# theivyzhang/droplet_visual_odometry

Hardware: AMD Instinct MI355X
Metric: frames/sec (detect+match+pose) at 1280×720, 2000 feats; ATE vs reference (higher is better)
Workload: dtype u8/f32/f64

## Files before the change

droplet_visual_odometry_amd/csrc/orb.hip:

```cpp
#include "dvo_internal.h"
#include "retain_best.h"

#include <climits>
#include <type_traits>

namespace dvo {

namespace {

__constant__ int8_t c_pattern[256 * 4] = {
#include "../../data/orb_bit_pattern_31.inc"
};
__constant__ __attribute__((aligned(16))) float c_pattern_f[256 * 4] = {
#include "../../data/orb_bit_pattern_31.inc"
};

constexpr int c_umax[16] = {15, 15, 15, 15, 14, 14, 14, 13, 13, 12, 11, 10, 9, 8, 6, 3};
struct IcTable {
    uint32_t w[4][32][10][2];
};
constexpr IcTable ic_table() {
    IcTable t{};
    for (int o = 0; o < 4; ++o)
        for (int r = 0; r < 31; ++r)
// ... 593 lines not shown
    const u16x2 Y = __builtin_elementwise_max(__builtin_elementwise_min(c0, c8), __builtin_elementwise_min(c4, c12));
    const u16x2 m = __builtin_elementwise_max(__builtin_elementwise_sub_sat(X, v), __builtin_elementwise_sub_sat(v, Y));
    return __builtin_bit_cast(uint32_t, __builtin_elementwise_sub_sat(m, as_u16x2(thr2)));
}
__device__ __forceinline__ uint32_t lane_prefix(unsigned long long bal) {
    return __builtin_amdgcn_mbcnt_hi((uint32_t)(bal >> 32), __builtin_amdgcn_mbcnt_lo((uint32_t)bal, 0u));
}
template <int kSeg>
__device__ __forceinline__ int seg_index(const int* cnt, int e) {
    int s = 0;
#pragma unroll
    for (int k = 0; k < 3; ++k) {
        const bool past = e >= cnt[k];
        e -= past ? cnt[k] : 0;
        s += past ? 1 : 0;
        if (!past) break;
    }
    return s * kSeg + e;
}
template <int kSeg>
__device__ __forceinline__ int seg_at(const uint16_t* list, const int* cnt, int e) {
    return list[seg_index<kSeg>(cnt, e)];
}
__global__ __launch_bounds__(kFastNT, DVO_FAST_WAVES_PER_EU) void fast_strip_kernel(StreamParams P, int nseg) {
    int it;
    const int f = xcd_frame_item(P.plan.total_strips * nseg, P.nframes, it);
    if (f >= P.nframes) return;
    const int strip = it / nseg, seg = it - strip * nseg;
    int l = 0;
    while (l + 1 < P.plan.nlevels && strip >= P.plan.L[l + 1].strip_base) ++l;
    const LevelGeom& G = P.plan.L[l];
    const int c = strip - G.strip_base;
    const int per_seg = (G.nbands + nseg - 1) / nseg;
    const int b_begin = seg * per_seg, b_end = min(G.nbands, b_begin + per_seg);
    if (b_begin >= b_end) return;
    const int w = G.w, h = G.h;
    const int xs = kBorder + c * kFastTW, xe = min(xs + kFastTW, w - kBorder);
    const int bx = xs - 7;
    const int thr = P.plan.fast_threshold;
    const uint8_t* src = level_ptr(P, f, l);
    const int sp = level_pitch(P, l);
    const auto rsrc = __builtin_amdgcn_make_buffer_rsrc(const_cast<uint8_t*>(src), 0, h * sp, 0x00020000);
    __shared__ __attribute__((aligned(16))) uint8_t img[kFtRows * kFtLW];
    __shared__ __attribute__((aligned(16))) uint8_t sc[(kBandRows + 2) * kFtLW];
    __shared__ uint16_t cand[4 * kFtSegCand + 256];
    __shared__ uint16_t wlist[4 * kFtWordCand + 256];
    __shared__ uint16_t carry[2][kFtCarryList];
    __shared__ int ncorner[4], ncarry[2];
    __shared__ uint32_t keep[kBandRows][4];
    __shared__ int row_off[4][kBandRows];
    const int lane = threadIdx.x & 63;
    const int wid = __builtin_amdgcn_readfirstlane(threadIdx.x >> 6);
    const int xlast = min(xe, w - 4);
    const int c_col = 4 + 4 * (lane & 31), c_hi = xlast - bx + 1 - c_col;
    const uint32_t c_vm = (c_col == 4 ? 0xFFFF0000u : 0xFFFFFFFFu) &
                          (c_hi >= 4 ? 0xFFFFFFFFu : c_hi <= 0 ? 0u : (1u << (8 * c_hi)) - 1u);
    const uint32_t c_vm4 = (c_vm & 1u) | ((c_vm >> 7) & 2u) | ((c_vm >> 14) & 4u) | ((c_vm >> 21) & 8u);
    const uint32_t thr2 = (uint32_t)thr * 0x10001u;
    uint32_t creg[kFtCarryR], pf[kFtPf], screg = 0;
    int voff[kFtPf];
#pragma unroll
    for (int k = 0; k < kFtPf; ++k) {
        const int q = threadIdx.x + k * kFastNT;
        const int rr = q / kFtWords, wd = q - rr * kFtWords;
        voff[k] = 4 * wd + rr * sp;
    }
    {
        const int ylo = kBorder + b_begin * kBandRows - 4;
#pragma unroll
        for (int k = 0; k < kFtCarryR; ++k) {
            const int q = threadIdx.x + k * kFastNT;
            creg[k] = q < kFtCarryW ? (uint32_t)__builtin_amdgcn_raw_buffer_load_b32(rsrc, voff[k], bx + ylo * sp, 0) : 0u;
        }
#pragma unroll
        for (int k = 0; k < kFtPf; ++k) {
            const int q = threadIdx.x + k * kFastNT;
            pf[k] = q < kFtNewW ? (uint32_t)__builtin_amdgcn_raw_buffer_load_b32(rsrc, voff[k], bx + (ylo + 8) * sp, 0) : 0u;
        }
    }
    if (threadIdx.x == 0) ncarry[0] = 0;
    for (int b = b_begin; b < b_end; ++b) {
        const int par = (b - b_begin) & 1;
        const int r0 = kBorder + b * kBandRows;
        const int r1 = min(r0 + kBandRows, h - kBorder);
        const int nrows = r1 - r0;
        const int item = G.band_base + b * G.ntx + c;
#pragma unroll
        for (int k = 0; k < kFtCarryR; ++k) {
            const int q = threadIdx.x + k * kFastNT;
            if (q < kFtCarryW) reinterpret_cast<uint32_t*>(img)[q] = creg[k];
        }
#pragma unroll
        for (int k = 0; k < kFtPf; ++k) {
            const int q = threadIdx.x + k * kFastNT;
            if (q < kFtNewW) reinterpret_cast<uint32_t*>(img)[kFtCarryW + q] = pf[k];
        }
        if (threadIdx.x < 2 * kFtWords) reinterpret_cast<uint32_t*>(sc)[threadIdx.x] = b == b_begin ? 0u : screg;
        for (int q = threadIdx.x; q < kBandRows * kFtLW / 16; q += kFastNT)
            reinterpret_cast<uint4*>(sc + 2 * kFtLW)[q] = make_uint4(0, 0, 0, 0);
        if (threadIdx.x < kBandRows * 4) keep[threadIdx.x >> 2][threadIdx.x & 3] = 0;
        if (threadIdx.x == 0) ncarry[par ^ 1] = 0;
        __syncthreads();
        if (b + 1 < b_end) {
#pragma unroll
            for (int k = 0; k < kFtCarryR; ++k) {
                const int q = threadIdx.x + k * kFastNT;
                creg[k] = q < kFtCarryW ? reinterpret_cast<const uint32_t*>(img)[kFtNewW + q] : 0u;
            }
            const int ynew = r0 + kBandRows + 4;
#pragma unroll
            for (int k = 0; k < kFtPf; ++k) {
                const int q = threadIdx.x + k * kFastNT;
                pf[k] = q < kFtNewW ? (uint32_t)__builtin_amdgcn_raw_buffer_load_b32(rsrc, voff[k], bx + ynew * sp, 0) : 0u;
            }
        }
        const int nsr = nrows + 2;
        const int sr_lo = b == b_begin ? 0 : 2;
        const int seg_off = wid * kFtSegCand, spare_i = 4 * kFtSegCand + wid * 64 + lane;
        int ncw = 0;
        {
            int n = 0, nw = 0;
            const int wl_off = wid * kFtWordCand, wl_spare = 4 * kFtWordCand + wid * 64 + lane;
            for (int sr = sr_lo + 2 * wid + (lane >> 5); __builtin_amdgcn_readfirstlane(sr - (lane >> 5)) < nsr;
                 sr += 8) {
                const int base = (sr + 3) * kFtLW + c_col;
                const uint32_t* wp = reinterpret_cast<const uint32_t*>(img + base);
                const uint32_t wc = wp[0], wl = wp[-1], wr = wp[1];
                const uint32_t wu = wp[-3 * kFtWords], wd = wp[3 * kFtWords];
                const uint32_t r0p = compass_pass(as_u16x2(__builtin_amdgcn_perm(0, wc, 0x0C020C00)),
                                                  as_u16x2(__builtin_amdgcn_perm(0, wu, 0x0C020C00)),
                                                  as_u16x2(__builtin_amdgcn_perm(0, wd, 0x0C020C00)),
                                                  as_u16x2(__builtin_amdgcn_perm(wr, wc, 0x0C050C03)),
                                                  as_u16x2(__builtin_amdgcn_perm(wc, wl, 0x0C030C01)), thr2);
                const uint32_t r1p = compass_pass(as_u16x2(__builtin_amdgcn_perm(0, wc, 0x0C030C01)),
                                                  as_u16x2(__builtin_amdgcn_perm(0, wu, 0x0C030C01)),
                                                  as_u16x2(__builtin_amdgcn_perm(0, wd, 0x0C030C01)),
                                                  as_u16x2(__builtin_amdgcn_perm(wr, wc, 0x0C060C04)),
                                                  as_u16x2(__builtin_amdgcn_perm(wc, wl, 0x0C040C02)), thr2);
                uint32_t b0, b1;
                asm("v_pk_min_u16 %0, %1, %2" : "=v"(b0) : "v"(r0p), "v"(0x00010001u));
                asm("v_pk_min_u16 %0, %1, %2" : "=v"(b1) : "v"(r1p), "v"(0x00010001u));
                const uint32_t m2 = b0 | (b1 << 1);
                const uint32_t msk = (m2 | (m2 >> 14)) & (sr < nsr ? c_vm4 : 0u);
                const bool any = msk != 0;
                const unsigned long long bal = __ballot(any);
                const int to = wl_off + nw + (int)lane_prefix(bal);
                wlist[any ? to : wl_spare] = (uint16_t)((base >> 2) | (msk << 12));
                nw += __popcll(bal);
            }
            __builtin_amdgcn_fence(__ATOMIC_RELEASE, "wavefront");
            __builtin_amdgcn_wave_barrier();
            __builtin_amdgcn_fence(__ATOMIC_ACQUIRE, "wavefront");
            for (int e0 = 0; e0 < nw; e0 += 64) {
                const int e = e0 + lane;
                const uint32_t ent = e < nw ? (uint32_t)wlist[wl_off + e] : 0u;
                const uint32_t msk = ent >> 12;
                const int a0 = (int)(ent & 0xFFFu) << 2;
                const uint32_t c = (uint32_t)__popc(msk);
                const unsigned long long b0 = __ballot(c & 1u), b1 = __ballot(c & 2u), b2 = __ballot(c & 4u);
                const int pre = n + (int)lane_prefix(b0) + 2 * (int)lane_prefix(b1) + 4 * (int)lane_prefix(b2);
#pragma unroll
                for (int k = 0; k < 4; ++k) {
                    const bool on = (msk >> k) & 1u;
                    const int to = seg_off + pre + __popc(msk & ((1u << k) - 1u));
                    if (on) cand[to] = (uint16_t)(a0 + k);
                }
                n += __popcll(b0) + 2 * __popcll(b1) + 4 * __popcll(b2);
            }
            __builtin_amdgcn_fence(__ATOMIC_RELEASE, "wavefront");
            __builtin_amdgcn_wave_barrier();
            __builtin_amdgcn_fence(__ATOMIC_ACQUIRE, "wavefront");
            for (int e0 = 0; e0 < n; e0 += 64) {
                const int e = e0 + lane;
                int a = 0, s = -1;
                if (e < n) {
                    a = cand[seg_off + e];
                    s = fast_score16_pk(img + a, kFtLW, thr);
                }
                const bool is_corner = s >= thr;
                if (is_corner) sc[a - 3 * kFtLW] = (uint8_t)s;
                const unsigned long long bal = __ballot(is_corner);
                cand[is_corner ? seg_off + ncw + (int)lane_prefix(bal) : spare_i] = (uint16_t)a;
                ncw += __popcll(bal);
            }
            if (lane == 0) ncorner[wid] = ncw;
        }
        __syncthreads();
        int cnt2[4];
#pragma unroll
        for (int k = 0; k < 4; ++k) cnt2[k] = ncorner[k];
        const int ncorners = cnt2[0] + cnt2[1] + cnt2[2] + cnt2[3];
        const int nc = ncarry[par];
        if (threadIdx.x < 2 * kFtWords) screg = reinterpret_cast<const uint32_t*>(sc)[kBandRows * kFtWords + threadIdx.x];
        for (int e = threadIdx.x; e < nc + ncorners; e += kFastNT) {
            const int a = (e < nc ? (int)carry[par][e] : seg_at<kFtSegCand>(cand, cnt2, e - nc)) -
                          3 * kFtLW;
            const int sr = a / kFtLW, x = bx + (a - sr * kFtLW);
            if (sr == kBandRows + 1) {
                const int slot = atomicAdd(&ncarry[par ^ 1], 1);
                carry[par ^ 1][slot] = (uint16_t)(a + 3 * kFtLW - kBandRows * kFtLW);
                continue;
            }
            if (sr < 1 || sr > nrows || x < xs || x >= xe) continue;
            const uint8_t* s = sc + a;
            const uint32_t v = s[0];
            const uint32_t nmax = max(max(max((uint32_t)s[-kFtLW - 1], (uint32_t)s[-kFtLW]),
                                          max((uint32_t)s[-kFtLW + 1], (uint32_t)s[-1])),
                                      max(max((uint32_t)s[1], (uint32_t)s[kFtLW - 1]),
                                          max((uint32_t)s[kFtLW], (uint32_t)s[kFtLW + 1])));
            if (v > nmax) {
                const int i_col = x - (xs - 1);
                atomicOr(&keep[sr - 1][i_col >> 5], 1u << (i_col & 31));
            }
        }
        __syncthreads();
        uint32_t* outp = P.buf.band_cand + (int64_t)f * P.plan.band_cand_stride + G.band_cand_off +
                         (int64_t)(b * G.ntx + c) * G.band_cap;
        {
            int rc = 0;
            if (lane < kBandRows && lane < nrows)
                rc = __popc(keep[lane][0]) + __popc(keep[lane][1]) + __popc(keep[lane][2]) + __popc(keep[lane][3]);
            int incl = rc;
#pragma unroll
            for (int o = 1; o < kBandRows; o <<= 1) {
                const int y2 = __shfl_up(incl, o);
                if (lane >= o) incl += y2;
            }
            if (lane < kBandRows) {
                row_off[wid][lane] = incl - rc;
                if (wid == 0)
                    P.buf.band_cnt[((int64_t)f * P.plan.total_bands + item) * kBandRows + lane] = ((incl - rc) << 16) | rc;
            }
            __builtin_amdgcn_fence(__ATOMIC_RELEASE, "wavefront");
            __builtin_amdgcn_wave_barrier();
            __builtin_amdgcn_fence(__ATOMIC_ACQUIRE, "wavefront");
        }
        for (int e = threadIdx.x; e < nc + ncorners; e += kFastNT) {
            const int a = (e < nc ? (int)carry[par][e] : seg_at<kFtSegCand>(cand, cnt2, e - nc)) - 3 * kFtLW;
            const int sr = a / kFtLW, x = bx + (a - sr * kFtLW);
            if (sr < 1 || sr > nrows || x < xs || x >= xe) continue;
            const int i_col = x - (xs - 1), wq = i_col >> 5;
            const uint32_t* kr = keep[sr - 1];
            if (!((kr[wq] >> (i_col & 31)) & 1)) continue;
            int before = __popc(kr[wq] & ((1u << (i_col & 31)) - 1));
            for (int q = 0; q < wq; ++q) before += __popc(kr[q]);
            outp[row_off[wid][sr - 1] + before] = ((uint32_t)sc[a] << 24) | ((uint32_t)(r0 + sr - 1) << 12) | (uint32_t)x;
        }
        __syncthreads();
    }
}

struct FastKeys {
    uint32_t* key;
    struct Elem {
        uint32_t k;
    };
    __device__ int val(int i) const { return (int)(key[i] >> 24); }
    __device__ void swap(int i, int j) const {
        uint32_t t = key[i];
        key[i] = key[j];
        key[j] = t;
    }
    __device__ Elem get(int i) const { return Elem{key[i]}; }
    __device__ void put(int i, Elem e) const { key[i] = e.k; }
    __device__ static int ev(Elem e) { return (int)(e.k >> 24); }
};

struct HarrisVals {
    float* v;
    uint32_t* key;
    struct Elem {
        float v;
        uint32_t k;
    };
    __device__ float val(int i) const { return v[i]; }
    __device__ void swap(int i, int j) const {
        float t = v[i];
        v[i] = v[j];
        v[j] = t;
        uint32_t u = key[i];
        key[i] = key[j];
        key[j] = u;
    }
    __device__ Elem get(int i) const { return Elem{v[i], key[i]}; }
    __device__ void put(int i, Elem e) const {
        v[i] = e.v;
        key[i] = e.k;
    }
    __device__ static float ev(Elem e) { return e.v; }
};

#ifndef DVO_SEL_NT
#define DVO_SEL_NT 128
#endif
constexpr int kSelNT = DVO_SEL_NT;
#ifndef DVO_SEL_NT0
#define DVO_SEL_NT0 256
#endif
constexpr int kSelNT0 = DVO_SEL_NT0;
#ifndef DVO_SEL_NT_CALL
#define DVO_SEL_NT_CALL 512
#endif
constexpr int kSelNTCall = DVO_SEL_NT_CALL, kSelCallFrames = 4;
constexpr int kSelLdsCap = 8192;
#ifndef DVO_SEL_LDS_CALL
#define DVO_SEL_LDS_CALL 1
#endif
constexpr bool kSelLdsCall = DVO_SEL_LDS_CALL != 0;

template <int NT, bool kLds>
__global__ __launch_bounds__(NT) void select_fast_kernel(StreamParams P, int l0) {
    const int l = l0 + blockIdx.x, f = blockIdx.y;
    if (l >= P.plan.nlevels) return;
    const LevelGeom& G = P.plan.L[l];
    __shared__ int lds[64];
    __shared__ int s_carry;
    const int32_t* rc = P.buf.band_cnt + ((int64_t)f * P.plan.total_bands + G.band_base) * kBandRows;
    const uint32_t* bsrc = P.buf.band_cand + (int64_t)f * P.plan.band_cand_stride + G.band_cand_off;
    uint32_t* A = P.buf.cand + (int64_t)f * P.plan.cand_stride + G.cand_off;
    if constexpr (kLds) {
        const int nseg = G.nbands * kBandRows * G.ntx;
        const int per = (nseg + NT - 1) / NT;
        const int s_begin = min(nseg, (int)threadIdx.x * per), s_end = min(nseg, s_begin + per);
        auto seg_word = [&](int sg) {
            const int cc = sg % G.ntx, br = sg / G.ntx;
            const int b = br / kBandRows, rr = br - b * kBandRows;
            const int tile = b * G.ntx + cc;
            return make_int2(tile, rc[(int64_t)tile * kBandRows + rr]);
        };
        constexpr int kG = 8;
        int mine = 0;
        for (int s0 = s_begin; s0 < s_end; s0 += kG) {
            int2 tv[kG];
#pragma unroll
            for (int k = 0; k < kG; ++k) tv[k] = s0 + k < s_end ? seg_word(s0 + k) : make_int2(0, 0);
#pragma unroll
            for (int k = 0; k < kG; ++k) mine += tv[k].y & 0xFFFF;
        }
        int tot;
        int o = block_excl_scan(mine, tot, lds);
        for (int s0 = s_begin; s0 < s_end; s0 += kG) {
            int2 tv[kG];
#pragma unroll
            for (int k = 0; k < kG; ++k) tv[k] = s0 + k < s_end ? seg_word(s0 + k) : make_int2(0, 0);
#pragma unroll
            for (int k = 0; k < kG; ++k) {
                const int cnt = tv[k].y & 0xFFFF, src_off = tv[k].x * G.band_cap + (tv[k].y >> 16);
                for (int i = 0; i < cnt; ++i) A[o + i] = bsrc[src_off + i];
                o += cnt;
            }
        }
        if (threadIdx.x == 0) s_carry = tot;
        __syncthreads();
    } else {
        const int nseg = G.nbands * kBandRows * G.ntx;
        if (threadIdx.x == 0) s_carry = 0;
        __syncthreads();
        for (int s0 = 0; s0 < nseg; s0 += NT) {
            const int sg = s0 + threadIdx.x;
            int cnt = 0, src_off = 0;
            if (sg < nseg) {
                const int cc = sg % G.ntx, br = sg / G.ntx;
                const int b = br / kBandRows, rr = br - b * kBandRows;
                const int tile = b * G.ntx + cc;
                const int v = rc[(int64_t)tile * kBandRows + rr];
                cnt = v & 0xFFFF;
                src_off = tile * G.band_cap + (v >> 16);
            }
            int tot;
            const int off = block_excl_scan(cnt, tot, lds);
            const int base = s_carry;
            for (int i = 0; i < cnt; ++i) A[base + off + i] = bsrc[src_off + i];
            __syncthreads();
            if (threadIdx.x == 0) s_carry = base + tot;
            __syncthreads();
        }
    }
    const int n = s_carry;
    __syncthreads();
    int32_t* Lpos = P.buf.sel_tmp + (int64_t)f * 2 * P.plan.cand_stride + 2 * G.cand_off;
    int32_t* Rasc = Lpos + G.cand_cap;
    int k;
    if constexpr (kLds) {
        __shared__ uint32_t s_key[kSelLdsCap];
        __shared__ int32_t s_L[kSelLdsCap], s_R[kSelLdsCap];
        if (n <= kSelLdsCap) {
            for (int i = threadIdx.x; i < n; i += NT) s_key[i] = A[i];
            __syncthreads();
            k = retain_best_block(FastKeys{s_key}, n, 2 * G.nper, -1, s_L, s_R, lds, P.plan.semantics);
            __syncthreads();
            for (int i = threadIdx.x; i < k; i += NT) A[i] = s_key[i];
        } else {
            k = retain_best_block(FastKeys{A}, n, 2 * G.nper, -1, Lpos, Rasc, lds, P.plan.semantics);
        }
    } else {
        k = retain_best_block(FastKeys{A}, n, 2 * G.nper, -1, Lpos, Rasc, lds, P.plan.semantics);
    }
    if (threadIdx.x == 0) P.buf.cnt1[f * kMaxLevels + l] = k;
}

#ifndef DVO_HARRIS_GROUPS
#define DVO_HARRIS_GROUPS 2
#endif
constexpr int kHG = DVO_HARRIS_GROUPS;
__host__ __device__ inline int harris_blocks_x(const Plan& pl) {
    int hb = 0;
    for (int l = 0; l < pl.nlevels; ++l) hb = hb > 2 * pl.L[l].nper ? hb : 2 * pl.L[l].nper;
    return (hb + 16 * kHG - 1) / (16 * kHG) + 1;
}

__global__ __launch_bounds__(256) void harris_kernel(StreamParams P) {
    __shared__ uint32_t win[kHG][16][32];
    const int l = blockIdx.y, f = blockIdx.z;
    const int hb = blockIdx.x, gdx = gridDim.x;
    const int n = P.buf.cnt1[f * kMaxLevels + l];
    const LevelGeom& G = P.plan.L[l];
    const uint8_t* img = level_ptr(P, f, l);
    const int step = level_pitch(P, l);
    const int lane = threadIdx.x & 63;
    const int wid = __builtin_amdgcn_readfirstlane(threadIdx.x >> 6);
    const int g = lane >> 4, j = lane & 15;
    const uint32_t* cand = P.buf.cand + (int64_t)f * P.plan.cand_stride + G.cand_off;
    float* resp = P.buf.resp + (int64_t)f * P.plan.cand_stride + G.cand_off;
    for (int base = (hb * 4 + wid) * 4 * kHG; base < n; base += gdx * 16 * kHG) {
        int x0[kHG], ax[kHG];
        uint32_t v0[kHG], v1[kHG];
#pragma unroll
        for (int u = 0; u < kHG; ++u) {
            const int i = min(base + 4 * u + g, n - 1);
            const uint32_t key = cand[i];
            x0[u] = key & 0xFFF;
            const int y0 = (key >> 12) & 0xFFF;
            ax[u] = (x0[u] - 4) & ~3;
            const uint8_t* wp = img + (int64_t)(y0 - 4) * step + ax[u];
            const int e1 = min(j + 16, 26);
            v0[u] = *reinterpret_cast<const uint32_t*>(wp + (int64_t)(j / 3) * step + 4 * (j % 3));
            v1[u] = *reinterpret_cast<const uint32_t*>(wp + (int64_t)(e1 / 3) * step + 4 * (e1 % 3));
        }
        __builtin_amdgcn_wave_barrier();
#pragma unroll
        for (int u = 0; u < kHG; ++u) {
            win[u][wid * 4 + g][j] = v0[u];
            win[u][wid * 4 + g][j + 16] = v1[u];
        }
        __builtin_amdgcn_wave_barrier();
#pragma unroll
        for (int u = 0; u < kHG; ++u) {
            const uint8_t* Wb = reinterpret_cast<const uint8_t*>(win[u][wid * 4 + g]);
            const int o = x0[u] - ax[u] - 3;
            int a = 0, b = 0, c = 0;
#pragma unroll
            for (int t = 0; t < 4; ++t) {
                const int pos = j + 16 * t;
                if (t < 3 || pos < 49) {
                    const int py = pos / 7, px = pos - 7 * py;
                    const uint8_t* q = Wb + (1 + py) * 12 + o + px;
                    const int Ix = (q[1] - q[-1]) * 2 + (q[-12 + 1] - q[-12 - 1]) + (q[12 + 1] - q[12 - 1]);
                    const int Iy = (q[12] - q[-12]) * 2 + (q[12 - 1] - q[-12 - 1]) + (q[12 + 1] - q[-12 + 1]);
                    a += Ix * Ix;
                    b += Iy * Iy;
                    c += Ix * Iy;
                }
            }
#pragma unroll
            for (int s2 = 8; s2 >= 1; s2 >>= 1) {
                a += __shfl_xor(a, s2);
                b += __shfl_xor(b, s2);
                c += __shfl_xor(c, s2);
            }
            if (j == 0 && base + 4 * u + g < n) {
                const float scale = 1.f / ((1 << 2) * 7 * 255.f);
                const float s4 = scale * scale * scale * scale;
                const float fa = (float)a, fb = (float)b, fc = (float)c;
                resp[base + 4 * u + g] = (fa * fb - fc * fc - 0.04f * (fa + fb) * (fa + fb)) * s4;
            }
        }
        __builtin_amdgcn_wave_barrier();
    }
}

template <int NT, bool kLds>
__global__ __launch_bounds__(NT) void select_harris_kernel(StreamParams P) {
    const int l = blockIdx.x, f = blockIdx.y;
    if (l >= P.plan.nlevels) return;
    const LevelGeom& G = P.plan.L[l];
    __shared__ int lds[64];
    const int n = P.buf.cnt1[f * kMaxLevels + l];
    uint32_t* A = P.buf.cand + (int64_t)f * P.plan.cand_stride + G.cand_off;
    float* R = P.buf.resp + (int64_t)f * P.plan.cand_stride + G.cand_off;
    int32_t* Lpos = P.buf.sel_tmp + (int64_t)f * 2 * P.plan.cand_stride + 2 * G.cand_off;
    int32_t* Rasc = Lpos + G.cand_cap;
    int k;
    if constexpr (kLds) {
        __shared__ float s_v[kSelLdsCap];
        __shared__ uint32_t s_key[kSelLdsCap];
        __shared__ int32_t s_L[kSelLdsCap], s_R[kSelLdsCap];
        if (n <= kSelLdsCap) {
            for (int i = threadIdx.x; i < n; i += NT) {
                s_v[i] = R[i];
                s_key[i] = A[i];
            }
            __syncthreads();
            k = retain_best_block(HarrisVals{s_v, s_key}, n, G.nper, -1, s_L, s_R, lds, P.plan.semantics);
            __syncthreads();
            for (int i = threadIdx.x; i < k; i += NT) {
                R[i] = s_v[i];
                A[i] = s_key[i];
            }
        } else {
            k = retain_best_block(HarrisVals{R, A}, n, G.nper, -1, Lpos, Rasc, lds, P.plan.semantics);
        }
    } else {
        k = retain_best_block(HarrisVals{R, A}, n, G.nper, -1, Lpos, Rasc, lds, P.plan.semantics);
    }
    if (threadIdx.x == 0) P.buf.cnt2[f * kMaxLevels + l] = k;
}

__device__ __forceinline__ float fast_atan2(float y, float x) {
    const float p1 = 0.9997878412794807f * (float)(180 / M_PI);
    const float p3 = -0.3258083974640975f * (float)(180 / M_PI);
    const float p5 = 0.1555786518463281f * (float)(180 / M_PI);
    const float p7 = -0.04432655554792128f * (float)(180 / M_PI);
    float ax = fabsf(x), ay = fabsf(y);
    float a, c, c2;
    if (ax >= ay) {
        c = ay / (ax + (float)2.220446049250313e-16);
        c2 = c * c;
        a = (((p7 * c2 + p5) * c2 + p3) * c2 + p1) * c;
    } else {
        c = ax / (ay + (float)2.220446049250313e-16);
        c2 = c * c;
        a = 90.f - (((p7 * c2 + p5) * c2 + p3) * c2 + p1) * c;
    }
    if (x < 0) a = 180.f - a;
    if (y < 0) a = 360.f - a;
    return a;
}

constexpr int kDPR = 19, kDPH = 2 * kDPR + 1, kDPW = 64;
#ifndef DVO_DKW
#define DVO_DKW 1
#endif
constexpr int kDKW = DVO_DKW;
constexpr int kDKB = 4 * kDKW;
constexpr int kICW = 36, kICR = 36;

constexpr int kDBRows = 8, kDBSeg = 5, kDBRaw = kDBRows + 6;
constexpr int kDBRow0 = 1;
constexpr int kDBBase[kDBSeg + 1] = {0, 11, 23, 35, 47, 56};
constexpr int kDBHalfW[kDBSeg] = {15, 18, 18, 18, 12};

__device__ __forceinline__ uint32_t sat_pk_u8(uint32_t v) {
    uint32_t d;
    asm("v_sat_pk_u8_i16 %0, %1" : "=v"(d) : "v"(v));
    return d;
}
__device__ __forceinline__ void describe_blur_rows(const uint32_t (&raw)[kDBRaw], uint8_t* patch_slot, int s, int wc,
                                                   bool st) {
    const u16x2 k18 = {18, 18}, k34 = {34, 34}, k49 = {49, 49}, k55 = {55, 55};
    const uint32_t R = 0x7FFFu;
    u16x2 lo[7], hi[7];
#pragma unroll
    for (int r = 0; r < kDBRaw; ++r) {
#pragma unroll
        for (int k = 0; k < 6; ++k) {
            lo[k] = lo[k + 1];
            hi[k] = hi[k + 1];
        }
        lo[6] = as_u16x2(__builtin_amdgcn_perm(0u, raw[r], 0x0C010C00u));
        hi[6] = as_u16x2(__builtin_amdgcn_perm(0u, raw[r], 0x0C030C02u));
        if (r < 6) continue;
        const u16x2 a = k18 * (lo[0] + lo[6]) + k34 * (lo[1] + lo[5]) + k49 * (lo[2] + lo[4]) + k55 * lo[3];
        const u16x2 b = k18 * (hi[0] + hi[6]) + k34 * (hi[1] + hi[5]) + k49 * (hi[2] + hi[4]) + k55 * hi[3];
        const uint32_t A = __builtin_bit_cast(uint32_t, a), B = __builtin_bit_cast(uint32_t, b);
        const u16x2 al = as_u16x2(dpp_from_left(A)), bl = as_u16x2(dpp_from_left(B));
        const u16x2 ar = as_u16x2(dpp_from_right(A)), br = as_u16x2(dpp_from_right(B));
        uint32_t s0 = __builtin_amdgcn_udot2(al, (u16x2){0, 18}, R, false);
        s0 = __builtin_amdgcn_udot2(bl, (u16x2){34, 49}, s0, false);
        s0 = __builtin_amdgcn_udot2(a, (u16x2){55, 49}, s0, false);
        s0 = __builtin_amdgcn_udot2(b, (u16x2){34, 18}, s0, false);
        uint32_t s1 = __builtin_amdgcn_udot2(bl, (u16x2){18, 34}, R, false);
        s1 = __builtin_amdgcn_udot2(a, (u16x2){49, 55}, s1, false);
        s1 = __builtin_amdgcn_udot2(b, (u16x2){49, 34}, s1, false);
        s1 = __builtin_amdgcn_udot2(ar, (u16x2){18, 0}, s1, false);
        uint32_t s2 = __builtin_amdgcn_udot2(bl, (u16x2){0, 18}, R, false);
        s2 = __builtin_amdgcn_udot2(a, (u16x2){34, 49}, s2, false);
        s2 = __builtin_amdgcn_udot2(b, (u16x2){55, 49}, s2, false);
        s2 = __builtin_amdgcn_udot2(ar, (u16x2){34, 18}, s2, false);
        uint32_t s3 = __builtin_amdgcn_udot2(a, (u16x2){18, 34}, R, false);
        s3 = __builtin_amdgcn_udot2(b, (u16x2){49, 55}, s3, false);
        s3 = __builtin_amdgcn_udot2(ar, (u16x2){49, 34}, s3, false);
        s3 = __builtin_amdgcn_udot2(br, (u16x2){18, 0}, s3, false);
        s0 += __builtin_amdgcn_ubfe(s0, 16, 1);
        s1 += __builtin_amdgcn_ubfe(s1, 16, 1);
        s2 += __builtin_amdgcn_ubfe(s2, 16, 1);
        s3 += __builtin_amdgcn_ubfe(s3, 16, 1);
        const uint32_t word = sat_pk_u8(__builtin_amdgcn_perm(s1, s0, 0x07060302u)) |
                              (sat_pk_u8(__builtin_amdgcn_perm(s3, s2, 0x07060302u)) << 16);
        const int i = kDBRow0 + kDBRows * s + (r - 6);
        if (st && s < kDBSeg && wc >= 1 && wc <= 11 && i < kDPH)
            reinterpret_cast<uint32_t*>(patch_slot + i * kDPW)[wc - 1] = word;
    }
}

template <int kCtl, int kRowMask = 0xF>
__device__ __forceinline__ int dpp_or_zero(int v) {
    return __builtin_amdgcn_update_dpp(0, v, kCtl, kRowMask, 0xF, false);
}
__device__ __forceinline__ int wave_sum_dpp(int v) {
    v += dpp_or_zero<0xB1>(v);
    v += dpp_or_zero<0x4E>(v);
    v += dpp_or_zero<0x114>(v);
    v += dpp_or_zero<0x118>(v);
    v += dpp_or_zero<0x142>(v);
    v += dpp_or_zero<0x143>(v);
    return __builtin_amdgcn_readlane(v, 63);
}

__global__ __launch_bounds__(256) void describe_kernel(StreamParams P) {
    __shared__ __attribute__((aligned(16))) uint8_t patch[kDKB][kDPH + 2][kDPW];
    __shared__ __attribute__((aligned(16))) uint8_t icw[4][kICR][kICW];
    __shared__ float s_ang[kDKB], s_ca[kDKB], s_sa[kDKB];
    __shared__ int s_pc[kDKB];
    const int nbx = (P.plan.kp_cap + kDKB - 1) / kDKB;
    int bxi;
    const int f = xcd_frame_item(nbx, P.nframes, bxi);
    if (f >= P.nframes) return;
    const int wv = __builtin_amdgcn_readfirstlane(threadIdx.x >> 6), lane = threadIdx.x & 63;
    const int32_t* c2 = P.buf.cnt2 + f * kMaxLevels;
    int cnt[kMaxLevels];
    int total = 0;
#pragma unroll
    for (int q = 0; q < kMaxLevels; ++q) {
        cnt[q] = q < P.plan.nlevels ? c2[q] : 0;
        total += cnt[q];
    }
    if (bxi == 0 && threadIdx.x == 0) {
        P.buf.nkp[f] = total;
        if (total > P.plan.kp_cap) atomicOr(&P.buf.status[f], 1);
    }
    const int nk = min(total, P.plan.kp_cap);
    if (bxi * kDKB >= nk) return;
    float4 pat[4];
#pragma unroll
    for (int q = 0; q < 4; ++q) pat[q] = reinterpret_cast<const float4*>(c_pattern_f)[q * 64 + lane];
    int lv[kDKW], ix[kDKW];
    uint32_t keys[kDKW];
    float resps[kDKW];
#pragma unroll
    for (int kk = 0; kk < kDKW; ++kk) {
        int l = 0, i = min(bxi * kDKB + wv * kDKW + kk, nk - 1);
#pragma unroll
        for (int q = 0; q + 1 < kMaxLevels; ++q)
            if (l == q && q + 1 < P.plan.nlevels && i >= cnt[q]) {
                i -= cnt[q];
                l = q + 1;
            }
        lv[kk] = l;
        ix[kk] = i;
        keys[kk] = P.buf.cand[(int64_t)f * P.plan.cand_stride + P.plan.L[l].cand_off + i];
        resps[kk] = P.buf.resp[(int64_t)f * P.plan.cand_stride + P.plan.L[l].cand_off + i];
    }
    constexpr int kIW = 31 * (kICW / 4);
    uint32_t ivs[kDKW][5], pvs[kDKW][kDBRaw];
    int db_s = 0;
#pragma unroll
    for (int q = 1; q < kDBSeg; ++q) db_s += lane >= kDBBase[q];
    const int db_k = lane - kDBBase[db_s];
    const int db_hw = db_s == 0 ? kDBHalfW[0] : db_s == 4 ? kDBHalfW[4] : kDBHalfW[1];
    const bool db_st = db_k >= 1 && db_k <= kDBBase[db_s + 1] - kDBBase[db_s] - 2;
    int db_wcs[kDKW];
#pragma unroll
    for (int kk = 0; kk < kDKW; ++kk) {
        const int l = lv[kk];
        const LevelGeom& G = P.plan.L[l];
        const uint32_t key = keys[kk];
        const int kx = key & 0xFFF, ky = (key >> 12) & 0xFFF;
        const float scale = G.scale;
        const float sc = 1.f / scale;
        const int cxb = cv_round_f((float)kx * scale * sc), cyb = cv_round_f((float)ky * scale * sc);
        const int a0 = (cxb - kDPR) & ~3;
        const int ai = (kx - 15) & ~3;
        const int step = level_pitch(P, l);
        const uint8_t* img = level_ptr(P, f, l) + (int64_t)(ky - 15) * step + ai;
#pragma unroll
        for (int t = 0; t < 5; ++t) {
            const int ec = min(64 * t + lane, kIW - 1);
            const int rc = ec / (kICW / 4), wc = ec - rc * (kICW / 4);
            ivs[kk][t] = *reinterpret_cast<const uint32_t*>(img + (int64_t)rc * step + 4 * wc);
        }
        {
            const int sr = min(db_s, kDBSeg - 1);
            const int db_wc = min(((cxb - db_hw - a0) >> 2) + db_k, 12);
            db_wcs[kk] = db_wc;
            const uint8_t* rw = level_ptr(P, f, l) + (int64_t)(cyb - kDPR - 3 + kDBRow0 + kDBRows * sr) * step +
                                a0 - 4 + 4 * db_wc;
#pragma unroll
            for (int t = 0; t < kDBRaw; ++t) pvs[kk][t] = *reinterpret_cast<const uint32_t*>(rw + (int64_t)t * step);
        }
    }
#pragma unroll
    for (int kk = 0; kk < kDKW; ++kk) {
        const int slot = wv * kDKW + kk;
        const int k = bxi * kDKB + slot;
        if (k >= nk) continue;
        const int l = lv[kk];
        const LevelGeom& G = P.plan.L[l];
        const uint32_t key = keys[kk];
        const int kx = key & 0xFFF, ky = (key >> 12) & 0xFFF;
        const float scale = G.scale;
        const float ptx = (float)kx * scale, pty = (float)ky * scale;
        const float sc = 1.f / scale;
        const int cxb = cv_round_f(ptx * sc);
        const int a0 = (cxb - kDPR) & ~3;
        const int ai = (kx - 15) & ~3;
        __builtin_amdgcn_wave_barrier();
#pragma unroll
        for (int t = 0; t < 5; ++t) reinterpret_cast<uint32_t*>(&icw[wv][0][0])[64 * t + lane] = ivs[kk][t];
        const int db_wc = db_wcs[kk];
        describe_blur_rows(pvs[kk], &patch[slot][0][0], db_s, db_wc, db_st);
        __builtin_amdgcn_wave_barrier();
        int m10, m01;
        {
            const int r = lane >> 1, hh = lane & 1;
            const uint32_t* rowp = reinterpret_cast<const uint32_t*>(&icw[wv][0][0]) + r * (kICW / 4) + 5 * hh;
            const uint2* tp = reinterpret_cast<const uint2*>(&c_ictab.w[(kx - 15) & 3][r][5 * hh][0]);
            uint32_t dU = 0, d1 = 0;
#pragma unroll
            for (int q = 0; q < 5; ++q) {
                const uint32_t I4 = rowp[q];
                const uint2 t = tp[q];
                dU = __builtin_amdgcn_udot4(I4, t.x, dU, false);
                d1 = __builtin_amdgcn_udot4(I4, t.y, d1, false);
            }
            m10 = (int)dU - 15 * (int)d1;
            m01 = (r - 15) * (int)d1;
        }
        (void)ai;
        m10 = wave_sum_dpp(m10);
        m01 = wave_sum_dpp(m01);
        if (lane == 0) {
            const float angle = fast_atan2((float)m01, (float)m10);
            s_ang[slot] = angle;
            s_pc[slot] = kDPR * kDPW + (cxb - a0);
            dvo_keypoint kp;
            kp.x = ptx;
            kp.y = pty;
            kp.size = 31 * scale;
            kp.angle = angle;
            kp.response = resps[kk];
            kp.octave = l;
            kp.class_id = -1;
            P.buf.kps[(int64_t)f * P.plan.kp_cap + k] = kp;
        }
        __builtin_amdgcn_wave_barrier();
    }
    __syncthreads();
    if (threadIdx.x < kDKB) {
        const float ang = s_ang[threadIdx.x] * (float)(M_PI / 180.f);
        double sd, cd;
        sincos((double)ang, &sd, &cd);
        s_ca[threadIdx.x] = (float)cd;
        s_sa[threadIdx.x] = (float)sd;
    }
    __syncthreads();
    constexpr float kRoundM = 12582912.0f;
    constexpr uint32_t kRoundC = 65u * 0x4B400000u;
    static_assert(sizeof(patch) < 65536, "patch offsets");
    const uint8_t* pbytes = &patch[0][0][0];
    for (int kk = 0; kk < kDKW; ++kk) {
        const int slot = wv * kDKW + kk;
        const int k = bxi * kDKB + slot;
        if (k >= nk) break;
        const float ca = s_ca[slot], sa = s_sa[slot];
        const uint32_t pc = (uint32_t)(slot * (kDPH + 2) * kDPW + s_pc[slot]) - kRoundC;
        typedef float f32x2 __attribute__((ext_vector_type(2)));
        const f32x2 cs = {ca, sa}, nsc = {-sa, ca};
        const auto at = [&](float px, float py) {
            const f32x2 r = (cs * (f32x2){px, px} + nsc * (f32x2){py, py}) + (f32x2){kRoundM, kRoundM};
            const uint32_t X = __float_as_uint(r.x), Y = __float_as_uint(r.y);
            return (uint32_t)pbytes[(Y << 6) + X + pc];
        };
        uint32_t t0[4], t1[4];
#pragma unroll
        for (int q = 0; q < 4; ++q) {
            t0[q] = at(pat[q].x, pat[q].y);
            t1[q] = at(pat[q].z, pat[q].w);
        }
        unsigned long long words[4];
#pragma unroll
        for (int q = 0; q < 4; ++q) words[q] = __ballot(t0[q] < t1[q]);
        if (lane < 4) {
            unsigned long long* d = reinterpret_cast<unsigned long long*>(P.buf.desc + ((int64_t)f * P.plan.kp_cap + k) * 32);
            d[lane] = lane == 0 ? words[0] : lane == 1 ? words[1] : lane == 2 ? words[2] : words[3];
        }
    }
}

__global__ void test_retain_best_kernel(float* resp, uint32_t* payload, int32_t* tmp, int n, int npoints, int depth,
                                        int semantics, int* kout) {
    __shared__ int lds[64];
    int k = retain_best_block(HarrisVals{resp, payload}, n, npoints, depth, tmp, tmp + n + 1, lds, semantics);
    if (threadIdx.x == 0) *kout = k;
}

}

hipError_t launch_blur(const StreamParams& P, hipStream_t s) {
    hipLaunchKernelGGL(blur_kernel, dim3(P.plan.total_tiles * xcd_frames(P.nframes)), dim3(256), 0, s, P);
    return hipGetLastError();
}


// ... 130 lines not shown
```

droplet_visual_odometry_amd/csrc/retain_best.h:

```cpp
#pragma once
#include <climits>

#include "dvo_internal.h"

namespace dvo {
namespace {

__device__ __forceinline__ void block_excl_scan2(int fa, int fb, int& pa, int& pb, int& ta, int& tb, int* lds) {
    const int lane = threadIdx.x & 63, wid = threadIdx.x >> 6, nw = blockDim.x >> 6;
    unsigned long long ma = __ballot(fa), mb = __ballot(fb);
    unsigned long long lt = lane == 0 ? 0ull : (~0ull >> (64 - lane));
    if (lane == 0) {
        lds[wid] = __popcll(ma);
        lds[32 + wid] = __popcll(mb);
    }
    __syncthreads();
    int oa = 0, ob = 0, sa = 0, sb = 0;
    for (int w = 0; w < nw; ++w) {
        int ca = lds[w], cb = lds[32 + w];
        if (w < wid) {
            oa += ca;
            ob += cb;
        }
        sa += ca;
        sb += cb;
    }
    __syncthreads();
    pa = oa + __popcll(ma & lt);
    pb = ob + __popcll(mb & lt);
    ta = sa;
    tb = sb;
}

__device__ __forceinline__ int block_sum(int v, int* lds) {
    const int lane = threadIdx.x & 63, wid = threadIdx.x >> 6, nw = blockDim.x >> 6;
#pragma unroll
    for (int o = 32; o > 0; o >>= 1) v += __shfl_xor(v, o);
    if (lane == 0) lds[wid] = v;
    __syncthreads();
    int s = 0;
    for (int w = 0; w < nw; ++w) s += lds[w];
    __syncthreads();
    return s;
}

template <class A, class V>
__device__ int partition_step(const A& a, int first, int last, V p, int32_t* Lpos, int32_t* Rasc, int* lds) {
    int nL = 0, nR = 0;
    for (int base = first; base < last; base += blockDim.x) {
        const int i = base + threadIdx.x;
        const bool in = i < last;
        V v = in ? a.val(i) : p;
        int fl = in && i >= first + 1 && !(v > p);
        int fr = in && !(p > v);
        int pa, pb, ta, tb;
        block_excl_scan2(fl, fr, pa, pb, ta, tb, lds);
        if (fl) Lpos[nL + pa] = i;
        if (fr) Rasc[nR + pb] = i;
        nL += ta;
        nR += tb;
    }
    __syncthreads();
    const int K = min(nL, nR);
    int cnt = 0;
    for (int k = threadIdx.x; k < K; k += blockDim.x) cnt += Lpos[k] < Rasc[nR - 1 - k];
    const int kstar = block_sum(cnt, lds);
    for (int k = threadIdx.x; k < kstar; k += blockDim.x) a.swap(Lpos[k], Rasc[nR - 1 - k]);
    const int cl = kstar < nL ? Lpos[kstar] : INT_MAX;
    const int cr = kstar > 0 ? Rasc[nR - kstar] : INT_MAX;
    __syncthreads();
    return min(cl, cr);
}

template <class A>
__device__ void adjust_heap(const A& a, int first, int hole, int len, typename A::Elem value) {
    const int top = hole;
    int second = hole;
    while (second < (len - 1) / 2) {
        second = 2 * (second + 1);
        if (a.val(first + second) > a.val(first + second - 1)) second--;
        a.put(first + hole, a.get(first + second));
        hole = second;
    }
    if ((len & 1) == 0 && second == (len - 2) / 2) {
        second = 2 * (second + 1);
        a.put(first + hole, a.get(first + second - 1));
        hole = second - 1;
    }
    int parent = (hole - 1) / 2;
    while (hole > top && a.val(first + parent) > A::ev(value)) {
        a.put(first + hole, a.get(first + parent));
        hole = parent;
        parent = (hole - 1) / 2;
    }
    a.put(first + hole, value);
}

template <class A>
__device__ void heap_select(const A& a, int first, int middle, int last) {
    const int len = middle - first;
    if (len >= 2) {
        int parent = (len - 2) / 2;
        while (true) {
            adjust_heap(a, first, parent, len, a.get(first + parent));
            if (parent == 0) break;
            parent--;
        }
    }
    for (int i = middle; i < last; ++i)
        if (a.val(i) > a.val(first)) {
            typename A::Elem v = a.get(i);
            a.put(i, a.get(first));
            adjust_heap(a, first, 0, len, v);
        }
}

template <class A>
__device__ void insertion_sort(const A& a, int first, int last) {
    if (first == last) return;
    for (int i = first + 1; i != last; ++i) {
        typename A::Elem v = a.get(i);
        if (A::ev(v) > a.val(first)) {
            for (int k = i; k > first; --k) a.put(k, a.get(k - 1));
            a.put(first, v);
        } else {
            int k = i;
            while (A::ev(v) > a.val(k - 1)) {
                a.put(k, a.get(k - 1));
                --k;
            }
            a.put(k, v);
        }
    }
}

template <class A>
__device__ void move_median_to_first(const A& a, int result, int x, int y, int z) {
    if (a.val(x) > a.val(y)) {
        if (a.val(y) > a.val(z)) a.swap(result, y);
        else if (a.val(x) > a.val(z)) a.swap(result, z);
        else a.swap(result, x);
    } else if (a.val(x) > a.val(z)) a.swap(result, x);
    else if (a.val(y) > a.val(z)) a.swap(result, z);
    else a.swap(result, y);
}

template <class A>
__device__ int retain_best_block(const A& a, int n, int npoints, int depth, int32_t* Lpos, int32_t* Rasc, int* lds,
                                 int semantics = kOcv4) {
    if (npoints < 0 || n <= npoints) return n;
    if (npoints == 0) return 0;
    const int nth = semantics == kOcv32 ? npoints : npoints - 1;
    int first = 0, last = n;
    if (depth < 0) depth = 2 * (31 - __clz(n));
    bool heap_done = false;
    while (last - first > 3) {
        if (depth == 0) {
            if (threadIdx.x == 0) {
                heap_select(a, first, nth + 1, last);
                a.swap(first, nth);
            }
            heap_done = true;
            break;
        }
        --depth;
        if (threadIdx.x == 0) move_median_to_first(a, first, first + 1, first + (last - first) / 2, last - 1);
        __syncthreads();
        auto p = a.val(first);
        const int cut = partition_step(a, first, last, p, Lpos, Rasc, lds);
        if (cut <= first || cut >= last) break;
        if (cut <= nth) first = cut;
        else last = cut;
    }
    if (!heap_done && threadIdx.x == 0) insertion_sort(a, first, last);
    __syncthreads();
    auto amb = a.val(npoints - 1);
    int nL = 0, nR = 0;
    for (int base = npoints; base < n; base += blockDim.x) {
        const int i = base + threadIdx.x;
        const bool in = i < n;
        int fl = 0, fr = 0;
        if (in) {
            bool pr = a.val(i) >= amb;
            fl = !pr;
            fr = pr;
        }
        int pa, pb, ta, tb;
        block_excl_scan2(fl, fr, pa, pb, ta, tb, lds);
        if (fl) Lpos[nL + pa] = i;
        if (fr) Rasc[nR + pb] = i;
        nL += ta;
        nR += tb;
    }
    __syncthreads();
    const int K = min(nL, nR);
    int cnt = 0;
    for (int k = threadIdx.x; k < K; k += blockDim.x) cnt += Lpos[k] < Rasc[nR - 1 - k];
    const int kstar = block_sum(cnt, lds);
    for (int k = threadIdx.x; k < kstar; k += blockDim.x) a.swap(Lpos[k], Rasc[nR - 1 - k]);
    __syncthreads();
    return npoints + nR;
}

}
}
```

Before: 102,800.

## Process multiple elements per thread in block partition scans and segment gather

Block-wide partition and retain steps now handle K elements per thread. Per-thread counts are combined through bit-sliced ballots, so there are fewer block scans and barriers per pass. The non-LDS segment gather also processes several segments per thread, drops the shared carry variable and its extra syncs, and prefetches the first few copied words. The default call sites use K=1 for the select kernels while other callers default to K=4. This adds register pressure and more complex indexing.

New measurement: 102,900 (median of 5 runs). Within noise of the previous version (+0.1%).

```diff
diff --git a/droplet_visual_odometry_amd/csrc/orb.hip b/droplet_visual_odometry_amd/csrc/orb.hip
--- a/droplet_visual_odometry_amd/csrc/orb.hip
+++ b/droplet_visual_odometry_amd/csrc/orb.hip
@@ -919,6 +919,16 @@
 #define DVO_SEL_NT_CALL 512
 #endif
 constexpr int kSelNTCall = DVO_SEL_NT_CALL, kSelCallFrames = 4;
+#ifndef DVO_SEL_K_CALL
+#define DVO_SEL_K_CALL 1
+#endif
+#ifndef DVO_SEL_SEG_K
+#define DVO_SEL_SEG_K 2
+#endif
+#ifndef DVO_SEL_COPY_U
+#define DVO_SEL_COPY_U 4
+#endif
+constexpr int kSelKCall = DVO_SEL_K_CALL, kSelSegK = DVO_SEL_SEG_K, kSelCopyU = DVO_SEL_COPY_U;
 constexpr int kSelLdsCap = 8192;
 #ifndef DVO_SEL_LDS_CALL
 #define DVO_SEL_LDS_CALL 1
@@ -931,10 +941,10 @@
     if (l >= P.plan.nlevels) return;
     const LevelGeom& G = P.plan.L[l];
     __shared__ int lds[64];
-    __shared__ int s_carry;
     const int32_t* rc = P.buf.band_cnt + ((int64_t)f * P.plan.total_bands + G.band_base) * kBandRows;
     const uint32_t* bsrc = P.buf.band_cand + (int64_t)f * P.plan.band_cand_stride + G.band_cand_off;
     uint32_t* A = P.buf.cand + (int64_t)f * P.plan.cand_stride + G.cand_off;
+    int n = 0;
     if constexpr (kLds) {
         const int nseg = G.nbands * kBandRows * G.ntx;
         const int per = (nseg + NT - 1) / NT;
@@ -967,33 +977,52 @@
                 o += cnt;
             }
         }
-        if (threadIdx.x == 0) s_carry = tot;
-        __syncthreads();
+        n = tot;
     } else {
         const int nseg = G.nbands * kBandRows * G.ntx;
-        if (threadIdx.x == 0) s_carry = 0;
-        __syncthreads();
-        for (int s0 = 0; s0 < nseg; s0 += NT) {
-            const int sg = s0 + threadIdx.x;
-            int cnt = 0, src_off = 0;
-            if (sg < nseg) {
+        for (int s0 = 0; s0 < nseg; s0 += kSelSegK * NT) {
+            const int sg0 = s0 + kSelSegK * (int)threadIdx.x;
+            int tile[kSelSegK], v[kSelSegK];
+            const int32_t* wp[kSelSegK];
+#pragma unroll
+            for (int j = 0; j < kSelSegK; ++j) {
+                const int sg = min(sg0 + j, nseg - 1);
                 const int cc = sg % G.ntx, br = sg / G.ntx;
                 const int b = br / kBandRows, rr = br - b * kBandRows;
-                const int tile = b * G.ntx + cc;
-                const int v = rc[(int64_t)tile * kBandRows + rr];
-                cnt = v & 0xFFFF;
-                src_off = tile * G.band_cap + (v >> 16);
+                tile[j] = b * G.ntx + cc;
+                wp[j] = rc + (int64_t)tile[j] * kBandRows + rr;
+            }
+            __builtin_amdgcn_sched_barrier(0);
+#pragma unroll
+            for (int j = 0; j < kSelSegK; ++j) v[j] = *wp[j];
+            __builtin_amdgcn_sched_barrier(0);
+            int mine = 0;
+#pragma unroll
+            for (int j = 0; j < kSelSegK; ++j) {
+                if (sg0 + j >= nseg) v[j] = 0;
+                mine += v[j] & 0xFFFF;
             }
             int tot;
-            const int off = block_excl_scan(cnt, tot, lds);
-            const int base = s_carry;
-            for (int i = 0; i < cnt; ++i) A[base + off + i] = bsrc[src_off + i];
-            __syncthreads();
-            if (threadIdx.x == 0) s_carry = base + tot;
-            __syncthreads();
-        }
-    }
-    const int n = s_carry;
+            int o = n + block_excl_scan(mine, tot, lds);
+            uint32_t kv[kSelSegK][kSelCopyU > 0 ? kSelCopyU : 1];
+#pragma unroll
+            for (int j = 0; j < kSelSegK; ++j) {
+                const int cnt = v[j] & 0xFFFF, src_off = cnt ? tile[j] * G.band_cap + (v[j] >> 16) : 0;
+#pragma unroll
+                for (int u = 0; u < kSelCopyU; ++u) kv[j][u] = bsrc[src_off + min(u, max(cnt - 1, 0))];
+            }
+#pragma unroll
+            for (int j = 0; j < kSelSegK; ++j) {
+                const int cnt = v[j] & 0xFFFF, src_off = tile[j] * G.band_cap + (v[j] >> 16);
+#pragma unroll
+                for (int u = 0; u < kSelCopyU; ++u)
+                    if (u < cnt) A[o + u] = kv[j][u];
+                for (int i = kSelCopyU; i < cnt; ++i) A[o + i] = bsrc[src_off + i];
+                o += cnt;
+            }
+            n += tot;
+        }
+    }
     __syncthreads();
     int32_t* Lpos = P.buf.sel_tmp + (int64_t)f * 2 * P.plan.cand_stride + 2 * G.cand_off;
     int32_t* Rasc = Lpos + G.cand_cap;
@@ -1004,11 +1033,11 @@
         if (n <= kSelLdsCap) {
             for (int i = threadIdx.x; i < n; i += NT) s_key[i] = A[i];
             __syncthreads();
-            k = retain_best_block(FastKeys{s_key}, n, 2 * G.nper, -1, s_L, s_R, lds, P.plan.semantics);
+            k = retain_best_block<kSelKCall>(FastKeys{s_key}, n, 2 * G.nper, -1, s_L, s_R, lds, P.plan.semantics);
             __syncthreads();
             for (int i = threadIdx.x; i < k; i += NT) A[i] = s_key[i];
         } else {
-            k = retain_best_block(FastKeys{A}, n, 2 * G.nper, -1, Lpos, Rasc, lds, P.plan.semantics);
+            k = retain_best_block<kSelKCall>(FastKeys{A}, n, 2 * G.nper, -1, Lpos, Rasc, lds, P.plan.semantics);
         }
     } else {
         k = retain_best_block(FastKeys{A}, n, 2 * G.nper, -1, Lpos, Rasc, lds, P.plan.semantics);
@@ -1118,14 +1147,14 @@
                 s_key[i] = A[i];
             }
             __syncthreads();
-            k = retain_best_block(HarrisVals{s_v, s_key}, n, G.nper, -1, s_L, s_R, lds, P.plan.semantics);
+            k = retain_best_block<kSelKCall>(HarrisVals{s_v, s_key}, n, G.nper, -1, s_L, s_R, lds, P.plan.semantics);
             __syncthreads();
             for (int i = threadIdx.x; i < k; i += NT) {
                 R[i] = s_v[i];
                 A[i] = s_key[i];
             }
         } else {
-            k = retain_best_block(HarrisVals{R, A}, n, G.nper, -1, Lpos, Rasc, lds, P.plan.semantics);
+            k = retain_best_block<kSelKCall>(HarrisVals{R, A}, n, G.nper, -1, Lpos, Rasc, lds, P.plan.semantics);
         }
     } else {
         k = retain_best_block(HarrisVals{R, A}, n, G.nper, -1, Lpos, Rasc, lds, P.plan.semantics);
diff --git a/droplet_visual_odometry_amd/csrc/retain_best.h b/droplet_visual_odometry_amd/csrc/retain_best.h
--- a/droplet_visual_odometry_amd/csrc/retain_best.h
+++ b/droplet_visual_odometry_amd/csrc/retain_best.h
@@ -6,28 +6,42 @@
 namespace dvo {
 namespace {
 
-__device__ __forceinline__ void block_excl_scan2(int fa, int fb, int& pa, int& pb, int& ta, int& tb, int* lds) {
+#ifndef DVO_SEL_K
+#define DVO_SEL_K 4
+#endif
+constexpr int kSelK = DVO_SEL_K;
+
+template <int K>
+__device__ __forceinline__ void block_excl_scan2(int ca, int cb, int& pa, int& pb, int& ta, int& tb, int* lds) {
     const int lane = threadIdx.x & 63, wid = threadIdx.x >> 6, nw = blockDim.x >> 6;
-    unsigned long long ma = __ballot(fa), mb = __ballot(fb);
-    unsigned long long lt = lane == 0 ? 0ull : (~0ull >> (64 - lane));
+    const unsigned long long lt = lane == 0 ? 0ull : (~0ull >> (64 - lane));
+    int wa = 0, wb = 0, xa = 0, xb = 0;
+#pragma unroll
+    for (int b = 0; (K >> b) != 0; ++b) {
+        const unsigned long long ma = __ballot((ca >> b) & 1), mb = __ballot((cb >> b) & 1);
+        wa += __popcll(ma) << b;
+        wb += __popcll(mb) << b;
+        xa += __popcll(ma & lt) << b;
+        xb += __popcll(mb & lt) << b;
+    }
     if (lane == 0) {
-        lds[wid] = __popcll(ma);
-        lds[32 + wid] = __popcll(mb);
+        lds[wid] = wa;
+        lds[32 + wid] = wb;
     }
     __syncthreads();
     int oa = 0, ob = 0, sa = 0, sb = 0;
     for (int w = 0; w < nw; ++w) {
-        int ca = lds[w], cb = lds[32 + w];
+        int va = lds[w], vb = lds[32 + w];
         if (w < wid) {
-            oa += ca;
-            ob += cb;
-        }
-        sa += ca;
-        sb += cb;
-    }
-    __syncthreads();
-    pa = oa + __popcll(ma & lt);
-    pb = ob + __popcll(mb & lt);
+            oa += va;
+            ob += vb;
+        }
+        sa += va;
+        sb += vb;
+    }
+    __syncthreads();
+    pa = oa + xa;
+    pb = ob + xb;
     ta = sa;
     tb = sb;
 }
@@ -44,26 +58,53 @@
     return s;
 }
 
-template <class A, class V>
-__device__ int partition_step(const A& a, int first, int last, V p, int32_t* Lpos, int32_t* Rasc, int* lds) {
-    int nL = 0, nR = 0;
-    for (int base = first; base < last; base += blockDim.x) {
-        const int i = base + threadIdx.x;
-        const bool in = i < last;
-        V v = in ? a.val(i) : p;
-        int fl = in && i >= first + 1 && !(v > p);
-        int fr = in && !(p > v);
+template <int K, class A, class Flag>
+__device__ __forceinline__ void collect_stops(const A& a, int begin, int end, Flag flag, int32_t* Lpos,
+                                              int32_t* Rasc, int* lds, int& nL, int& nR) {
+    nL = 0;
+    nR = 0;
+    for (int base = begin; base < end; base += K * blockDim.x) {
+        const int i0 = base + K * threadIdx.x;
+        decltype(a.val(0)) v[K];
+#pragma unroll
+        for (int j = 0; j < K; ++j) v[j] = a.val(min(i0 + j, end - 1));
+        unsigned ml = 0, mr = 0;
+#pragma unroll
+        for (int j = 0; j < K; ++j) {
+            bool fl, fr;
+            flag(i0 + j, v[j], fl, fr);
+            const bool in = i0 + j < end;
+            ml |= (unsigned)(fl & in) << j;
+            mr |= (unsigned)(fr & in) << j;
+        }
         int pa, pb, ta, tb;
-        block_excl_scan2(fl, fr, pa, pb, ta, tb, lds);
-        if (fl) Lpos[nL + pa] = i;
-        if (fr) Rasc[nR + pb] = i;
+        block_excl_scan2<K>(__popc(ml), __popc(mr), pa, pb, ta, tb, lds);
+        pa += nL;
+        pb += nR;
+#pragma unroll
+        for (int j = 0; j < K; ++j) {
+            if ((ml >> j) & 1) Lpos[pa++] = i0 + j;
+            if ((mr >> j) & 1) Rasc[pb++] = i0 + j;
+        }
         nL += ta;
         nR += tb;
     }
-    __syncthreads();
-    const int K = min(nL, nR);
+}
+
+template <int K, class A, class V>
+__device__ int partition_step(const A& a, int first, int last, V p, int32_t* Lpos, int32_t* Rasc, int* lds) {
+    int nL, nR;
+    collect_stops<K>(
+        a, first, last,
+        [&](int i, V v, bool& fl, bool& fr) {
+            fl = i >= first + 1 && !(v > p);
+            fr = !(p > v);
+        },
+        Lpos, Rasc, lds, nL, nR);
+    __syncthreads();
+    const int np = min(nL, nR);
     int cnt = 0;
-    for (int k = threadIdx.x; k < K; k += blockDim.x) cnt += Lpos[k] < Rasc[nR - 1 - k];
+    for (int k = threadIdx.x; k < np; k += blockDim.x) cnt += Lpos[k] < Rasc[nR - 1 - k];
     const int kstar = block_sum(cnt, lds);
     for (int k = threadIdx.x; k < kstar; k += blockDim.x) a.swap(Lpos[k], Rasc[nR - 1 - k]);
     const int cl = kstar < nL ? Lpos[kstar] : INT_MAX;
@@ -145,7 +186,7 @@
     else a.swap(result, y);
 }
 
-template <class A>
+template <int K = kSelK, class A>
 __device__ int retain_best_block(const A& a, int n, int npoints, int depth, int32_t* Lpos, int32_t* Rasc, int* lds,
                                  int semantics = kOcv4) {
     if (npoints < 0 || n <= npoints) return n;
@@ -167,7 +208,7 @@
         if (threadIdx.x == 0) move_median_to_first(a, first, first + 1, first + (last - first) / 2, last - 1);
         __syncthreads();
         auto p = a.val(first);
-        const int cut = partition_step(a, first, last, p, Lpos, Rasc, lds);
+        const int cut = partition_step<K>(a, first, last, p, Lpos, Rasc, lds);
         if (cut <= first || cut >= last) break;
         if (cut <= nth) first = cut;
         else last = cut;
@@ -175,27 +216,18 @@
     if (!heap_done && threadIdx.x == 0) insertion_sort(a, first, last);
     __syncthreads();
     auto amb = a.val(npoints - 1);
-    int nL = 0, nR = 0;
-    for (int base = npoints; base < n; base += blockDim.x) {
-        const int i = base + threadIdx.x;
-        const bool in = i < n;
-        int fl = 0, fr = 0;
-        if (in) {
-            bool pr = a.val(i) >= amb;
-            fl = !pr;
-            fr = pr;
-        }
-        int pa, pb, ta, tb;
-        block_excl_scan2(fl, fr, pa, pb, ta, tb, lds);
-        if (fl) Lpos[nL + pa] = i;
-        if (fr) Rasc[nR + pb] = i;
-        nL += ta;
-        nR += tb;
-    }
-    __syncthreads();
-    const int K = min(nL, nR);
+    int nL, nR;
+    collect_stops<K>(
+        a, npoints, n,
+        [&](int, decltype(amb) v, bool& fl, bool& fr) {
+            fr = v >= amb;
+            fl = !fr;
+        },
+        Lpos, Rasc, lds, nL, nR);
+    __syncthreads();
+    const int np = min(nL, nR);
     int cnt = 0;
-    for (int k = threadIdx.x; k < K; k += blockDim.x) cnt += Lpos[k] < Rasc[nR - 1 - k];
+    for (int k = threadIdx.x; k < np; k += blockDim.x) cnt += Lpos[k] < Rasc[nR - 1 - k];
     const int kstar = block_sum(cnt, lds);
     for (int k = threadIdx.x; k < kstar; k += blockDim.x) a.swap(Lpos[k], Rasc[nR - 1 - k]);
     __syncthreads();
```
